# amogkam/ray_lightning_accelerators

Hardware: AMD Instinct MI355X
Metric: samples/sec (whole node) + DDP scaling eff, MNISTClassifier at 1/2/4/8 workers (higher is better)
Workload: dtype bf16; 1 GPU; model=MNISTClassifier(784-32-64-10), global_batch=32, per_gpu_batch=32, parallelism=dp1, impl=native, accelerator=ddp, launch=single, optimizer=Adam, route=single, hip_graph_steps=21, step_kernel=one-launch, step_launch=hip-graph

## Files before the change

### ray_lightning_accelerators_amd/csrc/bindings.cpp

```cpp
#include <torch/extension.h>
#include <cstdlib>
#include <map>
#include <mutex>
#include <tuple>
#include <ATen/hip/impl/HIPGuardImplMasqueradingAsCUDA.h>
#include <ATen/hip/impl/HIPStreamMasqueradingAsCUDA.h>

#include "kernels.h"
#include "comm/xgmi.h"

namespace {

using at::Tensor;
using c10::optional;

hipStream_t cur_stream(const Tensor& t) {
  return at::hip::getCurrentHIPStreamMasqueradingAsCUDA(t.get_device()).stream();
}

void check_dev(const Tensor& t, const char* name, at::ScalarType dt) {
  TORCH_CHECK(t.is_cuda(), name, " must be a GPU tensor");
  TORCH_CHECK(t.is_contiguous(), name, " must be contiguous");
  TORCH_CHECK(t.scalar_type() == dt, name, " has dtype ", t.scalar_type(), ", expected ", dt);
}
// ... 984 lines not shown
  TORCH_CHECK(conv3x3_dgrad_bn_ok(N, H, W, Cr, Co), "conv3x3_dgrad_bn_plan: unsupported shape");
  const rla::Conv3x3Geom g = conv3x3_dgrad_geom(N, H, W, Cr, Co);
  const rla::Conv3x3Instance ins = rla::conv3x3_instance(g, false);
  return {g.tm, g.wpb, g.vrows, rla::conv3x3_pieces_per_thread(g), ins.nx, ins.fixed ? 1 : 0};
}

std::vector<int64_t> conv1x1_plan(int64_t M, int64_t K, int64_t N, bool bwd) {
  TORCH_CHECK(bwd ? rla::conv1x1_bn_bwd_ok(M, (int)K, (int)N) : rla::conv1x1_stats_ok(M, (int)K, (int)N),
              "conv1x1_plan: unsupported shape");
  const rla::Conv1x1Plan p = rla::conv1x1_stats_plan(M, (int)N, bwd);
  return {p.tnw, p.gy, p.gx, p.tiles_per_blk, rla::conv1x1_variant((int)K, p)};
}

int64_t stem_grid(int64_t N, int64_t H, int64_t W) {
  const rla::StemGeom g{(int)N, (int)H, (int)W, (int)((H - 1) / 2 + 1), (int)((W - 1) / 2 + 1)};
  TORCH_CHECK(rla::stem_ok(g), "stem_grid: unsupported shape");
  return rla::stem_grid(g);
}

Tensor dp_pack_roundtrip(Tensor x, int64_t tag) {
  TORCH_CHECK(x.is_cuda() && x.scalar_type() == at::kFloat && x.is_contiguous(), "x: contiguous fp32 on the GPU");
  Tensor y = at::empty_like(x);
  TORCH_CHECK(rla::dp_pack_roundtrip(x.data_ptr<float>(), y.data_ptr<float>(), x.numel(), (int)tag, cur_stream(x)) == 0,
              "dp_pack_roundtrip: bad arguments");
  return y;
}

}

PYBIND11_MODULE(TORCH_EXTENSION_NAME, m) {
  m.doc() = "gfx950 HIP kernels of ray_lightning_accelerators_amd";
  m.def("adam_step", &adam_step, "fused Adam over a flat fp32 arena");
  m.def("sgd_step", &sgd_step, "fused SGD (momentum/nesterov/wd) over a flat fp32 arena");
  m.def("multi_copy", &multi_copy, "multi-tensor copy/scale/cast via a chunk table");
  m.def("scale_", &scale_, "in-place scale of an fp32 arena");
  m.def("sumsq", &sumsq, "sum of squares of an fp32 arena");
  m.def("mlp_train_step", &mlp_train_step, "fused MNIST-MLP forward+backward(+Adam) step",
        py::arg("x_u8"), py::arg("x_f32"), py::arg("labels"), py::arg("order"), py::arg("counters"),
        py::arg("n_batches"), py::arg("B"), py::arg("L1"), py::arg("L2"), py::arg("params"),
        py::arg("grads"), py::arg("exp_avg"), py::arg("exp_avg_sq"), py::arg("stats"),
        py::arg("accumulate_grad"), py::arg("apply_adam"), py::arg("advance_step"), py::arg("lr"),
        py::arg("beta1"), py::arg("beta2"), py::arg("eps"), py::arg("weight_decay"), py::arg("lr_t"),
        py::arg("adamw"), py::arg("stamps") = py::none());
  m.def("mlp_eval", &mlp_eval, "fused MNIST-MLP forward + NLL/accuracy");
  m.def("mlp3", &mlp3, "fused MNIST-MLP step v3 (pipelined layer 1): kind 0 step, 1 head, 2 tail-grad, "
        "3 tail-adam, 4 prime, 5 step with the in-kernel xGMI exchange, 6 one-launch step (B <= 32)");
  m.def("dp_pack_roundtrip", &dp_pack_roundtrip, "packed DP exchange wire form of fp32 pairs, encoded + decoded");
  m.def("mlp3_hand_words", [](int64_t l1, int64_t l2) { return rla::mlp3_hand_words((int)l1, (int)l2); });
  m.def("mlp3_hand_layout", []() {
    const rla::MLP3HandLayout h = rla::mlp3_hand_layout();
    py::dict d;
    d["ack"] = h.ack; d["err"] = h.err; d["sat"] = h.sat; d["nonfinite"] = h.nonfinite;
    d["last_step"] = h.last_step; d["words"] = h.words;
    return d;
  });
  m.def("mlp3_h1_copies", [](int64_t l1) { return rla::mlp3_h1_copies((int)l1); },
        "H1pre copies per ring slot of the v3 step (the layer-1 partials' atomic fan-in is split over them)");
  m.def("mlp3_dp_area_floats", []() { return rla::comm::kDpUnitAreaFloats; },
        "aux receive-area stride (floats) of the one-launch step's packed / owner protocols");
  m.def("mlp_adam", &mlp_adam, "MLP arena Adam + bf16 shadow refresh (update=False: refresh only)");
  m.def("mlp_shadow_size", [](int64_t l1, int64_t l2) { return rla::mlp_shadow_layout((int)l1, (int)l2).total; });
  m.def("mlp_supported", [](int64_t a, int64_t b) { return rla::mlp_supported((int)a, (int)b); });
  m.def("mlp_param_count", &mlp_param_count);
  m.def("bn_partial", &bn_partial, "fused BN: per-block partial sums (mode 0 fwd stats, 1 bwd dz/dz*x)",
        py::arg("x"), py::arg("y"), py::arg("dy"), py::arg("C"), py::arg("mode"), py::arg("relu"), py::arg("nbt"),
        py::arg("dy2") = py::none(), py::arg("ss") = py::none(), py::arg("dout") = py::none(),
        py::arg("pool_arg") = py::none(), py::arg("pool_geo") = std::vector<int64_t>{});
  m.def("bn_finalize", &bn_finalize, "fused BN: mean/invstd/scale/shift + running stats from partials",
        py::arg("part"), py::arg("count"), py::arg("weight"), py::arg("bias"), py::arg("running_mean"),
        py::arg("running_var"), py::arg("nbt"), py::arg("momentum"), py::arg("eps"), py::arg("nbt_pending") = false);
  m.def("bn_bwd_finalize", &bn_bwd_finalize, "fused BN backward: dgamma/dbeta + dx coefficients");
  m.def("bn_apply", &bn_apply, "fused BN apply: y = act(x*scale + shift (+res))", py::arg("x"), py::arg("scale"),
        py::arg("shift"), py::arg("res"), py::arg("relu"), py::arg("y"), py::arg("nbt_inc") = py::none());
  m.def("conv1x1_stats", &conv1x1_stats, "1x1 conv forward on MFMA + BatchNorm partial sums of its output",
        py::arg("x"), py::arg("w"), py::arg("pre_ss") = py::none(), py::arg("nbt_inc") = py::none());
  m.def("conv1x1_pre_ok", [](int64_t M, int64_t K, int64_t N) { return rla::conv1x1_pre_ok(M, (int)K, (int)N); });
  m.def("conv1x1_bn_bwd", &conv1x1_bn_bwd,
        "1x1 conv input gradient fused with the previous BatchNorm's backward partial -> (d, part)");
  m.def("conv1x1_bn_bwd_ok", [](int64_t M, int64_t K, int64_t N) { return rla::conv1x1_bn_bwd_ok(M, (int)K, (int)N); });
  m.def("conv1x1_stats_ok", [](int64_t M, int64_t K, int64_t N) { return rla::conv1x1_stats_ok(M, (int)K, (int)N); });
  m.def("maxpool_fwd", &maxpool_fwd,
        "NHWC bf16 max pool -> (y, one-byte window argmax); bn_ss: pool bf16(relu(x * scale + shift)) instead",
        py::arg("x"), py::arg("k"), py::arg("s"), py::arg("pad"), py::arg("bn_ss") = py::none(),
        py::arg("nbt_inc") = py::none());
  m.def("strided_add_", &strided_add_, "d[:, :, ::s, ::s] += g in place over NHWC bf16 rows (fp32 add)");
  m.def("gap_bwd", &gap_bwd, "global average pool backward over NHWC rows (16-byte stores)");
  m.def("maxpool_bwd", &maxpool_bwd, "NHWC bf16 max pool backward (gather through the argmax bytes)");
  m.def("bn_bwd_apply", &bn_bwd_apply, "fused BN backward apply: dx (+ dres = relu-masked dy)", py::arg("x"),
        py::arg("y"), py::arg("dy"), py::arg("coef"), py::arg("relu"), py::arg("dx"), py::arg("dres"),
        py::arg("dy2") = py::none(), py::arg("ss") = py::none(), py::arg("pool_arg") = py::none(),
        py::arg("pool_geo") = std::vector<int64_t>{});
  m.def("conv_wgrad", &conv_wgrad, "NHWC bf16 conv weight gradient on MFMA -> fp32 [Cout, KH, KW, Cin]",
        py::arg("dy"), py::arg("x"), py::arg("N"), py::arg("H"), py::arg("W"), py::arg("Cin"), py::arg("OH"),
        py::arg("OW"), py::arg("Cout"), py::arg("KH"), py::arg("KW"), py::arg("sh"), py::arg("sw"), py::arg("ph"),
        py::arg("pw"), py::arg("splits") = 0, py::arg("algo") = 0, py::arg("pre_ss") = py::none());
  m.def("conv_wgrad_plan", &conv_wgrad_plan, "the wgrad kernel's (kind, wa, wb, splits, rows_per_split)",
        py::arg("N"), py::arg("H"), py::arg("W"), py::arg("Cin"), py::arg("OH"), py::arg("OW"), py::arg("Cout"),
        py::arg("KH"), py::arg("KW"), py::arg("sh"), py::arg("sw"), py::arg("ph"), py::arg("pw"),
        py::arg("splits") = 0, py::arg("algo") = 0);
  m.def("set_plan_cus", [](int64_t n) { rla::set_plan_cus((int)std::min<int64_t>(std::max<int64_t>(n, 0), 1 << 20)); },
        "pin the CU count the persistent conv kernels' work splits are planned for (process-wide; n <= 0: the "
        "device's); the tests use it to run production per-workgroup geometry on small tensors",
        py::arg("n"));
  m.def("plan_cus", []() { return (int64_t)rla::plan_cus(); }, "the effective planning CU count");
  m.def("conv3x3_plan", &conv3x3_plan, "the 3x3 kernel's (tm, wpb, vrows, pieces_per_thread, nx, fixed)", py::arg("N"),
        py::arg("H"), py::arg("W"), py::arg("Cin"), py::arg("Cout"), py::arg("flip") = false,
// ... 38 lines not shown
```

### ray_lightning_accelerators_amd/csrc/kernels.h

```cpp
#pragma once
#include <hip/hip_runtime.h>
#include <stdint.h>

namespace rla {

struct AdamArgs {
  float* p;
  const float* g;
  float* m;
  float* v;
  uint16_t* p_bf16;
  int64_t n;
  float lr, beta1, beta2, eps, weight_decay, grad_scale;
  int adamw, maximize;
  const int64_t* step_ptr;
  int64_t host_step;
  const float* lr_ptr;
};

struct SGDArgs {
  float* p;
  const float* g;
  float* buf;
  uint16_t* p_bf16;
// ... 143 lines not shown
  int B, L1, L2;
  const float* params;
  float* logits;
  float* out;
  int partials;
};

struct MLP3Args {
  const uint8_t* x_u8;
  const int64_t* labels;
  const int64_t* order;
  int64_t order_stride;
  int64_t* counters;
  int64_t n_batches;
  int B, L1, L2;
  float* params;
  float* grads;
  float* exp_avg;
  float* exp_avg_sq;
  uint16_t* shadow;
  uint16_t* dh1t;
  uint16_t* xring;
  int* h1pre;
  uint16_t* act;
  int* yring;
  float* stats;
  int stats_ring;
  float* head_part;
  int apply_adam;
  int advance_step;
  float lr, beta1, beta2, eps, weight_decay, grad_scale;
  const float* lr_ptr;
  int adamw;
  int64_t* stamps;
  char* dp_regions[8];
  uint32_t* dp_gen;
  int* dp_err;
  int64_t dp_stride;
  int64_t dp_spin;
  int dp_rank, dp_world;
  int dp_lite;
  int dp_proto;
  int dp_loop;
  unsigned long long* hand;
  int64_t hand_spin;
};
enum MLP3Kind { kMLP3Step = 0, kMLP3Head = 1, kMLP3TailGrad = 2, kMLP3TailAdam = 3, kMLP3Prime = 4,
                kMLP3StepDP = 5, kMLP3Step1 = 6, kMLP3Step1DP = 7 };
int64_t mlp3_hand_words(int L1, int L2);
struct MLP3HandLayout {
  int ack, err, sat, nonfinite, last_step, words;
};
MLP3HandLayout mlp3_hand_layout();
int launch_mlp3(const MLP3Args& a, int kind, hipStream_t stream);

int mlp3_act_rows(int L1, int L2);
int mlp3_h1_copies(int L1);
int dp_pack_roundtrip(const float* x, float* y, int64_t n, int tag, hipStream_t stream);

int launch_mlp_train_step(const MLPStepArgs& a, hipStream_t stream);
int launch_mlp_eval(const MLPEvalArgs& a, hipStream_t stream);
bool mlp_supported(int L1, int L2);
int launch_mlp_adam(const MLPAdamArgs& a, hipStream_t stream);

}

namespace rla {
struct WgradGeom {
  int N, H, W, Cin;
  int OH, OW, Cout;
  int KH, KW, sh, sw, ph, pw;
};
struct WgradPlan {
  int kind;
  int wa, wb;
  int splits;
  int64_t rows_per_split;
};
WgradPlan wgrad_plan(const WgradGeom& g, int splits, int algo = 0);
void launch_wgrad(const uint16_t* dy, const uint16_t* x, float* out, float* part, const WgradGeom& g,
                  const WgradPlan& p, hipStream_t stream, const float* pre_ss = nullptr);

struct Conv3x3Geom {
  int N, H, W, Cin, Cout;
  int vrows;
  int tm;
  int wpb;
};
int plan_cus();
void set_plan_cus(int n);
int conv3x3_wpb(int N, int H, int W, int Cout);
int conv3x3_pick_tm(int N, int H, int W, int Cout);
int conv3x3_vrows(const Conv3x3Geom& g);
int conv3x3_pieces_per_thread(const Conv3x3Geom& g);
bool conv3x3_ok(const Conv3x3Geom& g);
struct Conv3x3Instance {
  int nx;
  bool fixed;
};
Conv3x3Instance conv3x3_instance(const Conv3x3Geom& g, bool pre);
bool conv3x3_pre_ok(const Conv3x3Geom& g);
bool conv3x3_bwd_ok(const Conv3x3Geom& g);
bool launch_conv3x3(const uint16_t* x, const uint16_t* w, uint16_t* y, const Conv3x3Geom& g, bool flip,
                    hipStream_t stream, float* part = nullptr, const float* pre_ss = nullptr,
                    int64_t* nbt_inc = nullptr, const uint16_t* bwd_x = nullptr);

// ... 26 lines not shown
```

### ray_lightning_accelerators_amd/csrc/mlp_common.h

```cpp
#pragma once
#include <math.h>

#include "common.h"

namespace rla {
namespace mlp {

constexpr int kD = 784;
constexpr int kNC = 10;
constexpr int kTiles = kD / 16;

template <int L1, int L2>
struct Off {
  static constexpr int64_t W1 = 0, B1 = (int64_t)L1 * kD, W2 = B1 + L1, B2 = W2 + (int64_t)L2 * L1,
                           W3 = B2 + L2, B3 = W3 + kNC * L2, NP = B3 + kNC;
  static constexpr int64_t W2T = (NP + 7) / 8 * 8, W3T = W2T + (int64_t)L1 * L2;
};

struct AdamScal {
  float lr, step_size, bc2_sqrt, beta1, beta2, eps, wd;
  int adamw;
};

__device__ __forceinline__ void adam_scalars(AdamScal& o, int64_t t, float lr, float b1, float b2, float eps,
                                             float wd, int adamw) {
  const double bc1 = 1.0 - pow((double)b1, (double)t);
  const double bc2 = 1.0 - pow((double)b2, (double)t);
  o.lr = lr;
  o.step_size = (float)((double)lr / bc1);
  o.bc2_sqrt = (float)sqrt(bc2);
  o.beta1 = b1; o.beta2 = b2; o.eps = eps; o.wd = wd; o.adamw = adamw;
}

__device__ __forceinline__ float adam1(float p, float g, float& m, float& v, const AdamScal& o) {
#pragma clang fp contract(off)
  if (o.wd != 0.f) {
    if (o.adamw) p = p * (1.f - o.lr * o.wd);
    else g = fmaf(o.wd, p, g);
  }
  m = fmaf(1.f - o.beta1, g - m, m);
  v = fmaf(1.f - o.beta2, g * g, v * o.beta2);
  const float denom = sqrtf(v) / o.bc2_sqrt + o.eps;
  return fmaf(-o.step_size, m / denom, p);
}

typedef __attribute__((address_space(3))) bf16x4 lds_bf16x4;
__device__ __forceinline__ bf16x4 tr_read(const __bf16* p) {
  return __builtin_amdgcn_ds_read_tr16_b64_v4bf16((lds_bf16x4*)(p));
}
__device__ __forceinline__ bf16x8 ld8(const __bf16* p) { return *reinterpret_cast<const bf16x8*>(p); }
__device__ __forceinline__ float4 ld4(const float* p) { return *reinterpret_cast<const float4*>(p); }

__device__ __forceinline__ void u8x16_to_bf16(const uint4 v, bf16x8& lo, bf16x8& hi) {
  const uint32_t wd[4] = {v.x, v.y, v.z, v.w};
  constexpr float inv255 = 1.0f / 255.0f;
#pragma unroll
  for (int j = 0; j < 4; ++j) {
    lo[j] = (__bf16)((float)((wd[0] >> (8 * j)) & 0xffu) * inv255);
    lo[4 + j] = (__bf16)((float)((wd[1] >> (8 * j)) & 0xffu) * inv255);
    hi[j] = (__bf16)((float)((wd[2] >> (8 * j)) & 0xffu) * inv255);
    hi[4 + j] = (__bf16)((float)((wd[3] >> (8 * j)) & 0xffu) * inv255);
  }
}

}
}
```

### ray_lightning_accelerators_amd/csrc/mlp_step3.hip

```cpp
#include <cfloat>

#include "common.h"
#include "kernels.h"
#include "mlp_common.h"
#include "comm/xgmi.h"

namespace rla {
namespace {

using namespace mlp;
using comm::kDpMaxBlocks;
using comm::kXgmiFlagBytes;
using comm::kXgmiMaxRanks;

constexpr int kThreads = 512;
constexpr int kWaves = 8;
constexpr int kDZS = 40;
constexpr int kXSS = 24;
constexpr int kBMax = 256;
constexpr int kCnt = 5;
constexpr int kHeadRows = 32;

enum TailMode { kFused = 0, kGrad = 1, kAdam = 2, kPrime = 3, kFusedDP = 4 };

// ... 24 lines not shown
};

template <int BC, int L1, int L2>
constexpr bool fits3() {
  return Cfg3<BC, L1, L2>::total + 256 <= 160 * 1024;
}

__device__ __forceinline__ __bf16 relu_bf(float x) { return (__bf16)fmaxf(x, 0.f); }

constexpr float kFix = 1048576.0f;
constexpr float kFixSat = 33554432.0f;
__device__ __forceinline__ unsigned f32_to_fixed(float x) {
  return (unsigned)__float2int_rn(fminf(fmaxf(x * kFix, -kFixSat), kFixSat));
}
__device__ __forceinline__ float fixed_to_f32(int q) { return (float)q * (1.0f / 1048576.0f); }

template <int L1>
struct H1Copies {
  static constexpr int G = L1 <= 64 ? 2 : 1;
};

__device__ __forceinline__ void gather_tile(const MLP3Args& a, int kt, int64_t ob, int64_t cursor,
                                            int64_t dst_slot, int nthreads) {
  const int tid = threadIdx.x;
  const int B = a.B, Bp = (B + 31) / 32 * 32;
  const int64_t* idx = a.order + ob * a.order_stride + cursor * B;
  __bf16* dst = reinterpret_cast<__bf16*>(a.xring) + (dst_slot * kTiles + kt) * (int64_t)Bp * 16;
  for (int b = tid; b < Bp; b += nthreads) {
    bf16x8 lo = zero8(), hi = zero8();
    if (b < B) u8x16_to_bf16(*reinterpret_cast<const uint4*>(a.x_u8 + idx[b] * kD + kt * 16), lo, hi);
    *reinterpret_cast<bf16x8*>(dst + b * 16) = lo;
    *reinterpret_cast<bf16x8*>(dst + b * 16 + 8) = hi;
  }
  if (kt == 0)
    for (int b = tid; b < Bp; b += nthreads) a.yring[dst_slot * Bp + b] = b < B ? (int)a.labels[idx[b]] : -1;
}

__device__ __forceinline__ int64_t ld_state(const int64_t* p, int i) {
  return ((const __attribute__((address_space(4))) int64_t*)(p))[i];
}

__device__ __forceinline__ void stamp_max(const MLP3Args& a, int k) {
  if (a.stamps && threadIdx.x == 0)
    atomicMax(reinterpret_cast<unsigned long long*>(a.stamps + k),
              (unsigned long long)__builtin_amdgcn_s_memrealtime());
}

constexpr int kSeq = 10;
constexpr int kHandAck = 0, kHandErr = 16, kHandWords = 32;

constexpr int kHandSat = 17, kHandNonFinite = 18, kHandLastStep = 19;
static_assert(kHandLastStep < kHandWords, "health words inside the hand buffer");
constexpr float kH1Sat = 32.0f;

struct H1Health {
  unsigned sat = 0u, bad = 0u;
};

__device__ __forceinline__ void h1_check(H1Health& h, const f32x4& d, int row0, int B) {
  const bool trouble = !(fabsf(d[0]) <= kH1Sat) | !(fabsf(d[1]) <= kH1Sat) | !(fabsf(d[2]) <= kH1Sat) |
                       !(fabsf(d[3]) <= kH1Sat);
  if (__builtin_amdgcn_ballot_w64(trouble) == 0ull) return;
#pragma unroll
  for (int i = 0; i < 4; ++i) {
    const float m = fabsf(d[i]);
    const bool real = row0 + i < B, finite = m <= FLT_MAX;
    h.bad += (unsigned)__builtin_popcountll(__builtin_amdgcn_ballot_w64(real && !finite));
    h.sat += (unsigned)__builtin_popcountll(__builtin_amdgcn_ballot_w64(real && finite && m > kH1Sat));
  }
}

__device__ __forceinline__ void h1_report(const MLP3Args& a, const H1Health& h, int64_t step) {
  if ((h.sat | h.bad) == 0u || !a.hand) return;
  if ((threadIdx.x & 63) == 0) {
    if (h.sat)
      __hip_atomic_fetch_add(a.hand + kHandSat, (unsigned long long)h.sat, __ATOMIC_RELAXED, __HIP_MEMORY_SCOPE_AGENT);
    if (h.bad)
      __hip_atomic_fetch_add(a.hand + kHandNonFinite, (unsigned long long)h.bad, __ATOMIC_RELAXED,
                             __HIP_MEMORY_SCOPE_AGENT);
    __hip_atomic_fetch_max(a.hand + kHandLastStep, (unsigned long long)step, __ATOMIC_RELAXED,
                           __HIP_MEMORY_SCOPE_AGENT);
  }
}

struct RepPre {
  bool active;
  int64_t si;
  int kt;
  uint4 xn;
  int64_t yn;
  uint32_t raw;
};

struct NoHook {
  __device__ void operator()() const {}
};

__device__ __forceinline__ void dma_lds16(const void* gsrc, uint32_t lds) {
  uint32_t keep;
  asm volatile("s_mov_b32 %0, m0\n\ts_mov_b32 m0, %2\n\ts_nop 0\n\tglobal_load_lds_dwordx4 %1, off\n\ts_mov_b32 m0, %0"
               : "=&s"(keep)
               : "v"(gsrc), "s"(lds)
               : "memory");
}
__device__ __forceinline__ void dma_lds4(const void* gsrc, uint32_t lds) {
  uint32_t keep;
// ... 558 lines not shown
      row = REP ? L->dh2t + (e - L1) * L->ts : ACT + (int64_t)(A::DH2T + e - L1) * Bp;
      r.gi[0] = O::B2 + (e - L1);
    } else {
      row = REP ? L->dzt + (e - L1 - L2) * L->ts : ACT + (int64_t)(A::DZT + e - L1 - L2) * Bp;
      r.gi[0] = O::B3 + (e - L1 - L2);
    }
    if (setup) {
      r.kind = 2;
      r.valid[0] = true;
      if (prefetch_adam) { r.pv[0] = a.params[r.gi[0]]; r.mv[0] = a.exp_avg[r.gi[0]]; r.vv[0] = a.exp_avg_sq[r.gi[0]]; }
    }
    if (!compute) return;
    float s8[8] = {0.f, 0.f, 0.f, 0.f, 0.f, 0.f, 0.f, 0.f};

    for (int b0 = 0; b0 < Bp; b0 += 32) {
      bf16x8 v[4];
#pragma unroll
      for (int q = 0; q < 4; ++q) v[q] = ld8(row + b0 + 8 * q);
#pragma unroll
      for (int q = 0; q < 4; ++q)
#pragma unroll
        for (int j = 0; j < 8; ++j) s8[j] += (float)v[q][j];
    }
    r.v[0] = ((s8[0] + s8[1]) + (s8[2] + s8[3])) + ((s8[4] + s8[5]) + (s8[6] + s8[7]));
  }
}

template <int L1, int L2>
__device__ __forceinline__ void small_finalize(const MLP3Args& a, bool adam, const SmallRes& r, const AdamScal& o) {
  using O = Off<L1, L2>;
  if (r.kind < 0) return;
  __bf16* SHW = reinterpret_cast<__bf16*>(a.shadow);
  bf16x4 sh4;
#pragma unroll
  for (int i = 0; i < 4; ++i) {
    sh4[i] = (__bf16)0.f;
    if (!r.valid[i]) continue;
    if (adam) {
      float m_ = r.mv[i], v_ = r.vv[i];
      const float p_ = adam1(r.pv[i], r.v[i], m_, v_, o);
      a.params[r.gi[i]] = p_;
      a.exp_avg[r.gi[i]] = m_;
      a.exp_avg_sq[r.gi[i]] = v_;
      SHW[r.gi[i]] = (__bf16)p_;
      sh4[i] = (__bf16)p_;
    } else {
      a.grads[r.gi[i]] = r.v[i];
    }
  }
  if (adam && r.kind == 0) *reinterpret_cast<bf16x4*>(SHW + O::W2T + (int64_t)r.colv * L2 + r.rowv) = sh4;
  if (adam && r.kind == 1) *reinterpret_cast<bf16x4*>(SHW + O::W3T + (int64_t)r.colv * 16 + r.rowv) = sh4;
}

template <int L1, int L2>
__device__ __forceinline__ void small_store(const MLP3Args& a, const SmallRes& r, bool store_mv) {
  using O = Off<L1, L2>;
  if (r.kind < 0) return;
  __bf16* SHW = reinterpret_cast<__bf16*>(a.shadow);
  bf16x4 sh4;
#pragma unroll
  for (int i = 0; i < 4; ++i) {
    sh4[i] = (__bf16)0.f;
    if (!r.valid[i]) continue;
    a.params[r.gi[i]] = r.v[i];
    if (store_mv) {
      a.exp_avg[r.gi[i]] = r.mv[i];
      a.exp_avg_sq[r.gi[i]] = r.vv[i];
    }
    SHW[r.gi[i]] = (__bf16)r.v[i];
    sh4[i] = (__bf16)r.v[i];
  }
  if (r.kind == 0) *reinterpret_cast<bf16x4*>(SHW + O::W2T + (int64_t)r.colv * L2 + r.rowv) = sh4;
  if (r.kind == 1) *reinterpret_cast<bf16x4*>(SHW + O::W3T + (int64_t)r.colv * 16 + r.rowv) = sh4;
}

__device__ __forceinline__ uint32_t* dp_flag(char* region, int slot, int blk, int src) {
  return reinterpret_cast<uint32_t*>(region) + ((size_t)slot * kDpMaxBlocks + blk) * kXgmiMaxRanks + src;
}
__device__ __forceinline__ float* dp_data(char* region, int slot, int src, int64_t stride) {
  return reinterpret_cast<float*>(region + kXgmiFlagBytes) + ((int64_t)slot * kXgmiMaxRanks + src) * stride;
}

__device__ __forceinline__ int dp_begin(const MLP3Args& a, uint32_t* sh_gen) {
  if (threadIdx.x == 0) *sh_gen = a.dp_gen[blockIdx.x] + 1u;
  __syncthreads();
  return (int)(*sh_gen & 1u);
}

__device__ __forceinline__ void dp_signal_and_wait(const MLP3Args& a, uint32_t gen, int slot, int* sh_fail) {
  if (a.dp_lite) {
    const int tid = threadIdx.x, blk = blockIdx.x;
    asm volatile("s_waitcnt vmcnt(0)" ::: "memory");
    __syncthreads();
    if (tid < 64) {
      if (tid == 0) *sh_fail = 0;
      __builtin_amdgcn_fence(__ATOMIC_RELEASE, "");
      asm volatile("s_waitcnt vmcnt(0)" ::: "memory");
      if (tid < a.dp_world)
        __hip_atomic_store(dp_flag(a.dp_regions[tid], slot, blk, a.dp_rank), gen, __ATOMIC_RELAXED,
                           __HIP_MEMORY_SCOPE_SYSTEM);
      if (tid < a.dp_world) {
        uint32_t* f = dp_flag(a.dp_regions[a.dp_rank], slot, blk, tid);
        int64_t spins = 0;
        while (__hip_atomic_load(f, __ATOMIC_RELAXED, __HIP_MEMORY_SCOPE_SYSTEM) != gen) {
          if (++spins > a.dp_spin) {
            *sh_fail = 1;
// ... 542 lines not shown
  static constexpr int NSMALL = (NTASK + kWaves - 1) / kWaves;
  static constexpr size_t oImg = C::total;
  static constexpr size_t oTile = oImg + (size_t)(2 * L2 + L1) * C::TS * 2;
  static constexpr size_t oRaw = oTile + (size_t)(2 * 32 + L1) * kXSS * 2 + 64;
  static constexpr size_t lds = oRaw + kPreRawBytes;
};
static_assert(One<128, 256>::lds <= 160 * 1024, "one-launch LDS budget");

__device__ __forceinline__ void one_wait_acks(const MLP3Args& a, int64_t seq, int* sh_fail) {
  if (threadIdx.x == 0) {
    const long long target = (long long)(seq + 1) * (long long)gridDim.x;
    const long long* ack = reinterpret_cast<const long long*>(a.hand + kHandAck);
    int64_t n = 0;
    *sh_fail = 0;
    while (__hip_atomic_load(ack, __ATOMIC_RELAXED, __HIP_MEMORY_SCOPE_AGENT) < target) {
      if (++n > a.hand_spin) {
        *sh_fail = 1;
        __hip_atomic_store(a.hand + kHandErr, 1ull, __ATOMIC_RELAXED, __HIP_MEMORY_SCOPE_AGENT);
        if (a.dp_err) __hip_atomic_store(a.dp_err, 2, __ATOMIC_RELAXED, __HIP_MEMORY_SCOPE_SYSTEM);
        break;
      }
      __builtin_amdgcn_s_sleep(2);
    }
  }
  asm volatile("" ::: "memory");
  __syncthreads();
}

template <int L1, int L2, int DPP, int NW = 8>
__global__ __launch_bounds__(kThreads) void mlp3_one_kernel(MLP3Args a) {
  constexpr bool DP = DPP >= 0;
  using C = typename One<L1, L2>::C;
  using S = SmallTasks<L1, L2>;
  constexpr int TN1 = L1 / 16, Bp = 32;
  __shared__ __attribute__((aligned(16))) char smem[One<L1, L2>::lds];
  __shared__ int sh_fail;
  __bf16* sH2T = (__bf16*)(smem + One<L1, L2>::oImg);
  __bf16* sDH2T = sH2T + L2 * C::TS;
  __bf16* sDH1T = sDH2T + L2 * C::TS;
  __bf16* sX = (__bf16*)(smem + One<L1, L2>::oTile);
  __bf16* sXn = sX + Bp * kXSS;
  __bf16* sW = sXn + Bp * kXSS;
  AdamScal* sh_o = reinterpret_cast<AdamScal*>(sW + L1 * kXSS);
  const int tid = threadIdx.x, lane = tid & 63, w = tid >> 6, r16 = lane & 15, g = lane >> 4;
  const int blk = blockIdx.x;
  const bool tile = blk >= 1 && blk <= kTiles, small = blk > kTiles;
  const int kt = blk - 1;
  if (a.stamps && blk == 1 && tid == 0) a.stamps[8] = __builtin_amdgcn_s_memrealtime();
  stamp_max(a, 13);

  const int64_t c0 = ld_state(a.counters, 0), cursor = ld_state(a.counters, 1);
  const int64_t slot = ld_state(a.counters, 3), ob = ld_state(a.counters, 4);
  const int64_t seq = ld_state(a.counters, kSeq);
  const uint32_t dgen = DP ? dp_gen_now(a) : 0u;
  const int B = a.B;

  const int m = w * 16 + r16, pix = kt * 16 + 4 * g;
  const bool mw = tile && w < TN1;
  const int64_t gidx = mw ? (int64_t)m * kD + pix : 0;
  F4 p4, m4, v4;
  SmallRes r;
  r.kind = -1;
  const int task = (blk - 1 - kTiles) * kWaves + w;
  if (small) small_compute<L1, L2, true>(a, true, task, r);
  const float lr_now = a.lr_ptr ? ((const __attribute__((address_space(4))) float*)(a.lr_ptr))[0] : a.lr;
  __bf16* XR = reinterpret_cast<__bf16*>(a.xring);
  constexpr int64_t tile_elems = (int64_t)Bp * 16;
  const int xb = lane & 31;
  bf16x8 xc0, xc1;
  RepPre pre;
  pre.active = tile && w == PreWave<L1>::wave;
  pre.raw = (uint32_t)(uintptr_t)(const __attribute__((address_space(3))) void*)(smem + One<L1, L2>::oRaw);
  pre.kt = tile ? kt : 0;
  pre.xn = make_uint4(0u, 0u, 0u, 0u);
  pre.yn = -1;
  int64_t nc = cursor + 1, nob = ob;
  if (nc >= a.n_batches) { nc = 0; nob ^= 1; }
  const int kt_c = tile ? kt : 0;
  auto hook = [&]() {
    pre.si = a.order[nob * a.order_stride + nc * B + (xb < B ? xb : 0)];
    const __bf16* cur = XR + (slot * kTiles + kt_c) * tile_elems + xb * 16;
    xc0 = ld8(cur);
    xc1 = ld8(cur + 8);
    p4 = *reinterpret_cast<const F4*>(a.params + gidx);
    m4 = *reinterpret_cast<const F4*>(a.exp_avg + gidx);
    v4 = *reinterpret_cast<const F4*>(a.exp_avg_sq + gidx);
  };
  if (tid == 0 && blk > 0)
    adam_scalars(*sh_o, a.advance_step ? c0 + 1 : c0, lr_now, a.beta1, a.beta2, a.eps, a.weight_decay, a.adamw);

  head_body<32, L1, L2, false, true>(a, smem, &pre, hook);

  if (a.stamps && blk == 1 && tid == 0) a.stamps[9] = __builtin_amdgcn_s_memrealtime();
  stamp_max(a, 12);

  if (tile) {
    if (w == 0 && lane < 32) {
      *reinterpret_cast<bf16x8*>(sX + xb * kXSS) = xc0;
      *reinterpret_cast<bf16x8*>(sX + xb * kXSS + 8) = xc1;
    }
    __syncthreads();
    if (a.stamps && blk == 1 && tid == 0) a.stamps[7] = __builtin_amdgcn_s_memrealtime();
    bf16x4 w4;
    f32x4 acc = {0.f, 0.f, 0.f, 0.f};
    if (mw) {
      const int q = r16 >> 2, pp = r16 & 3;
      const bf16x4 lo = tr_read(sX + (8 * g + q) * kXSS + 4 * pp);
      const bf16x4 hi = tr_read(sX + (8 * g + 4 + q) * kXSS + 4 * pp);
      const bf16x8 afrag = __builtin_shufflevector(lo, hi, 0, 1, 2, 3, 4, 5, 6, 7);
      acc = mfma16(afrag, ld8(sDH1T + m * C::TS + 8 * g), acc);
    }
    bool adam_done = false, store_mv = true;
    if constexpr (DP) {
      const uint32_t gen = dgen;
      const int dslot = (int)(gen & 1u);
      int fail = 0;
      if (mw) {
        if constexpr (DPP == 0) {
#pragma unroll
          for (int i = 0; i < 4; ++i) dp_push_gran(a, dslot, gidx + i, acc[i], gen);
#pragma unroll
          for (int i = 0; i < 4; ++i) acc[i] = dp_sum_gran(a, dslot, gidx + i, gen, &fail) * a.grad_scale;
        } else {
          float v[4] = {acc[0], acc[1], acc[2], acc[3]};
          const int unit = blk * kWaves + w;
          if constexpr (DPP == 1) {
            dp_packed_exchange<NW>(a, unit, gen, v, a.grad_scale, &fail);
          } else {
            const AdamScal o = *sh_o;
            store_mv = dp_owner_step<NW>(a, unit, dp_task_owner(a, kt), gen, v, a.grad_scale, &fail,
                                     [&](float (&x)[4]) {
#pragma unroll
                                       for (int i = 0; i < 4; ++i) x[i] = adam1(p4.v[i], x[i], m4.v[i], v4.v[i], o);
                                     });
            store_mv = store_mv || a.dp_loop;
            adam_done = true;
#pragma unroll
            for (int i = 0; i < 4; ++i) p4.v[i] = v[i];
          }
#pragma unroll
          for (int i = 0; i < 4; ++i) acc[i] = v[i];
        }
      }
// ... 39 lines not shown
    if (mw) {
      constexpr int G = H1Copies<L1>::G;
      unsigned* h1 = reinterpret_cast<unsigned*>(a.h1pre + ((slot ^ 1) * G + kt % G) * (int64_t)Bp * L1);
      const bf16x8 bfrag = (g < 2) ? ld8(sW + (w * 16 + r16) * kXSS + 8 * g) : zero8();
      H1Health health;
#pragma unroll
      for (int mt = 0; mt < Bp / 16; ++mt) {
        const bf16x8 afrag = (g < 2) ? ld8(sXn + (mt * 16 + r16) * kXSS + 8 * g) : zero8();
        const f32x4 d = mfma16(afrag, bfrag, f32x4{0.f, 0.f, 0.f, 0.f});
        unsigned* dst = h1 + (int64_t)((mt * TN1 + w) * 4) * 64 + lane;
#pragma unroll
        for (int i = 0; i < 4; ++i) atomicAdd(dst + i * 64, f32_to_fixed(d[i]));
        h1_check(health, d, mt * 16 + 4 * g, B);
      }
      h1_report(a, health, c0 + 1);
    }
    if (a.stamps && blk == 1 && tid == 0) a.stamps[10] = __builtin_amdgcn_s_memrealtime();
    stamp_max(a, 5);
  } else if (small) {
    const RepLds L{(const __bf16*)(smem + C::oH1T), sH2T, sDH2T, (const __bf16*)(smem + C::odZT), sDH1T, C::TS};
    small_compute<L1, L2, true>(a, true, task, r, &L);
    bool adam_done = false, store_mv = true;
    if constexpr (DP) {
      const uint32_t gen = dgen;
      const int dslot = (int)(gen & 1u);
      int fail = 0;
      if constexpr (DPP == 0) {
#pragma unroll
        for (int i = 0; i < 4; ++i)
          if (r.valid[i]) dp_push_gran(a, dslot, r.gi[i], r.v[i], gen);
#pragma unroll
        for (int i = 0; i < 4; ++i)
          if (r.valid[i]) r.v[i] = dp_sum_gran(a, dslot, r.gi[i], gen, &fail) * a.grad_scale;
      } else if (task < S::NTASK) {
        float v[4] = {r.v[0], r.v[1], r.v[2], r.v[3]};
        const int unit = blk * kWaves + w;
        if constexpr (DPP == 1) {
          dp_packed_exchange<NW>(a, unit, gen, v, a.grad_scale, &fail);
        } else {
          const AdamScal o = *sh_o;
          store_mv = dp_owner_step<NW>(a, unit, dp_task_owner(a, kTiles + task), gen, v, a.grad_scale, &fail,
                                   [&](float (&x)[4]) {
#pragma unroll
                                     for (int i = 0; i < 4; ++i) x[i] = adam1(r.pv[i], x[i], r.mv[i], r.vv[i], o);
                                   });
          store_mv = store_mv || a.dp_loop;
          adam_done = true;
        }
#pragma unroll
        for (int i = 0; i < 4; ++i) r.v[i] = v[i];
      }
      dp_end_nosync(a, gen, fail);
    }
    one_wait_acks(a, seq, &sh_fail);
    if (adam_done) small_store<L1, L2>(a, r, store_mv);
    else small_finalize<L1, L2>(a, true, r, *sh_o);
    stamp_max(a, 6);
  } else {
    HeadStats hs{0.f, 0.f, 0.f};
    if (w == 0) hs = head_stats((const float*)(smem + C::oZ));
    one_wait_acks(a, seq, &sh_fail);
    uint4* z = reinterpret_cast<uint4*>(a.h1pre + slot * H1Copies<L1>::G * (int64_t)Bp * L1);
    for (int i = tid; i < H1Copies<L1>::G * Bp * L1 / 4; i += kThreads) z[i] = make_uint4(0u, 0u, 0u, 0u);
    if (tid == 0) {
      const int64_t t = c0 + 1;
      int64_t nc = cursor + 1, nob = ob;
      if (nc >= a.n_batches) { nc = 0; nob ^= 1; }
      const int64_t st[kCnt] = {a.advance_step ? t : t - 1, nc, cursor, slot ^ 1, nob};
      for (int k = 0; k < kCnt; ++k) a.counters[k] = a.counters[kCnt + k] = st[k];
      a.counters[kSeq] = seq + 1;
      if (a.stats) {
        float* sr = a.stats + (int)((t - 1) % (a.stats_ring > 0 ? a.stats_ring : 1)) * 4;
        sr[0] = hs.loss * (1.f / (float)B);
        sr[1] = hs.correct;
        sr[2] = hs.cnt;
        sr[3] = (float)t;
      }
      if (a.stamps) a.stamps[4] = __builtin_amdgcn_s_memrealtime();
    }
  }
  stamp_max(a, 11);
}

template <int L1, int L2>
int dispatch3(const MLP3Args& a, int kind, hipStream_t stream) {
  constexpr int kOneGrid = 1 + kTiles + One<L1, L2>::NSMALL;
  if (kind == kMLP3Step1) {
    if (a.B > 32 || !a.hand || kOneGrid > 256) return -5;
    hipLaunchKernelGGL((mlp3_one_kernel<L1, L2, -1>), dim3(kOneGrid), dim3(kThreads), 0, stream, a);
    return 0;
  }
  if (kind == kMLP3Step1DP) {
    if (a.B > 32 || !a.hand || kOneGrid > kDpMaxBlocks || a.dp_world < 1 || a.dp_world > kXgmiMaxRanks ||
        !a.dp_gen || !a.dp_err || a.dp_proto < 0 || a.dp_proto > 2)
      return -6;
    if (a.dp_proto == 0 ? (a.dp_lite != 2 || a.dp_stride < 2 * Off<L1, L2>::NP) : a.dp_stride < comm::kDpUnitAreaFloats)
      return -7;
    const dim3 g(kOneGrid), b(kThreads);
    const int nw = a.dp_world <= 2 ? 2 : (a.dp_world <= 4 ? 4 : 8);
    if (a.dp_proto == 0) hipLaunchKernelGGL((mlp3_one_kernel<L1, L2, 0>), g, b, 0, stream, a);
    else if (a.dp_proto == 1 && nw == 2) hipLaunchKernelGGL((mlp3_one_kernel<L1, L2, 1, 2>), g, b, 0, stream, a);
    else if (a.dp_proto == 1 && nw == 4) hipLaunchKernelGGL((mlp3_one_kernel<L1, L2, 1, 4>), g, b, 0, stream, a);
    else if (a.dp_proto == 1) hipLaunchKernelGGL((mlp3_one_kernel<L1, L2, 1, 8>), g, b, 0, stream, a);
    else if (nw == 2) hipLaunchKernelGGL((mlp3_one_kernel<L1, L2, 2, 2>), g, b, 0, stream, a);
    else if (nw == 4) hipLaunchKernelGGL((mlp3_one_kernel<L1, L2, 2, 4>), g, b, 0, stream, a);
    else hipLaunchKernelGGL((mlp3_one_kernel<L1, L2, 2, 8>), g, b, 0, stream, a);
    return 0;
  }
  constexpr int NT = 64 * (L1 / 16);
  if (kind == kMLP3StepDP && (a.dp_world < 1 || a.dp_world > kXgmiMaxRanks || !a.dp_gen || !a.dp_err ||
                              a.dp_stride < Off<L1, L2>::NP || kTiles + SmallTasks<L1, L2>::NBLK > kDpMaxBlocks))
    return -3;
  if (kind == kMLP3Step || kind == kMLP3Head || kind == kMLP3StepDP) {
    const int nchunks = (a.B + kHeadRows - 1) / kHeadRows;
    if (nchunks > 1 && !a.head_part) return -4;
    if (nchunks > 1)
      hipLaunchKernelGGL((mlp3_head_kernel<kHeadRows, L1, L2, true>), dim3(nchunks + kTiles), dim3(kThreads), 0, stream, a);
    else
      hipLaunchKernelGGL((mlp3_head_kernel<kHeadRows, L1, L2, false>), dim3(1 + kTiles), dim3(kThreads), 0, stream, a);
  }
  int mode = -1, grid = kTiles;
  if (kind == kMLP3Step) { mode = kFused; grid += SmallTasks<L1, L2>::NBLK; }
  else if (kind == kMLP3StepDP) { mode = kFusedDP; grid += SmallTasks<L1, L2>::NBLK; }
  else if (kind == kMLP3TailGrad) { mode = kGrad; grid += SmallTasks<L1, L2>::NBLK; }
  else if (kind == kMLP3Prime) mode = kPrime;
  else if (kind == kMLP3TailAdam) {
    mode = kAdam;
    const int64_t nsmall = Off<L1, L2>::NP - Off<L1, L2>::B1;
    int extra = (int)((nsmall + NT - 1) / NT);
    grid += extra < 64 ? extra : 64;
  }
  if (mode >= 0) hipLaunchKernelGGL((mlp3_tail_kernel<L1, L2>), dim3(grid), dim3(NT), 0, stream, a, mode);
  return 0;
}

static_assert(fits3<kHeadRows, 128, 256>(), "v3 head LDS budget");

__global__ void dp_pack_roundtrip_kernel(const float* x, float* y, int64_t n, uint32_t tag) {
  const int64_t i = (int64_t)blockIdx.x * blockDim.x + threadIdx.x;
  if (2 * i + 1 < n + 1) {
    const float v0 = x[2 * i], v1 = 2 * i + 1 < n ? x[2 * i + 1] : 0.f;
    const u64 w = pk2(v0, v1, tag);
    y[2 * i] = ((uint32_t)w & 3u) == tag ? pk_lo(w) : __builtin_nanf("");
    if (2 * i + 1 < n) y[2 * i + 1] = pk_hi(w);
  }
}

}

int dp_pack_roundtrip(const float* x, float* y, int64_t n, int tag, hipStream_t stream) {
  if (n <= 0 || tag < 0 || tag > 3) return -1;
  const int64_t pairs = (n + 1) / 2;
  hipLaunchKernelGGL(dp_pack_roundtrip_kernel, dim3((unsigned)((pairs + 255) / 256)), dim3(256), 0, stream, x, y, n,
                     (uint32_t)tag);
  return 0;
}

int mlp3_act_rows(int L1, int L2) { return L1 + 2 * L2 + 16; }
int mlp3_h1_copies(int L1) { return L1 <= 64 ? H1Copies<64>::G : H1Copies<128>::G; }
int64_t mlp3_hand_words(int, int) { return kHandWords; }
MLP3HandLayout mlp3_hand_layout() {
  return {kHandAck, kHandErr, kHandSat, kHandNonFinite, kHandLastStep, kHandWords};
}

int launch_mlp3(const MLP3Args& a, int kind, hipStream_t stream) {
  if (a.B > kBMax || a.B < 1) return -2;
#define RLA_CASE(a1, a2) if (a.L1 == a1 && a.L2 == a2) return dispatch3<a1, a2>(a, kind, stream);
  RLA_CASE(32, 32) RLA_CASE(32, 64) RLA_CASE(32, 128) RLA_CASE(32, 256)
  RLA_CASE(64, 64) RLA_CASE(64, 128) RLA_CASE(64, 256)
  RLA_CASE(128, 64) RLA_CASE(128, 128) RLA_CASE(128, 256)
#undef RLA_CASE
  return -1;
}

}
```

### ray_lightning_accelerators_amd/ops/fused_mlp.py

```python
from __future__ import annotations

import math
from typing import Dict, Optional, Sequence, Tuple

import torch
import torch.nn.functional as F

from . import require, use_native

IN_FEATURES = 784
NUM_CLASSES = 10
SUPPORTED = {(32, 32), (32, 64), (32, 128), (32, 256), (64, 64), (64, 128), (64, 256),
             (128, 64), (128, 128), (128, 256)}


def mlp_param_count(L1: int, L2: int) -> int:
    return L1 * IN_FEATURES + L1 + L2 * L1 + L2 + NUM_CLASSES * L2 + NUM_CLASSES


def mlp_supported(L1: int, L2: int) -> bool:
    return (int(L1), int(L2)) in SUPPORTED


def mlp_unpack(flat: torch.Tensor, L1: int, L2: int) -> Dict[str, torch.Tensor]:
# ... 101 lines not shown
def mlp_shadow_layout(L1: int, L2: int) -> Dict[str, int]:
    np_ = mlp_param_count(L1, L2)
    w2t = (np_ + 7) // 8 * 8
    w3t = w2t + L1 * L2
    return {"np": np_, "w2t": w2t, "w3t": w3t, "total": w3t + 16 * L2}


def mlp_refresh_shadow(params: torch.Tensor, shadow: torch.Tensor, L1: int, L2: int) -> None:
    if use_native(params):
        require().mlp_adam(params, params, params, params, shadow, int(L1), int(L2), 0.0, 0.9, 0.999, 1e-8, 0.0,
                           1.0, False, False, None, None)
        return
    lay = mlp_shadow_layout(L1, L2)
    v = mlp_unpack(params, L1, L2)
    with torch.no_grad():
        shadow[: lay["np"]].copy_(params)
        shadow[lay["w2t"]: lay["w3t"]].copy_(v["layer_2.weight"].t().reshape(-1))
        w3t = torch.zeros(L2, 16, dtype=params.dtype, device=params.device)
        w3t[:, :NUM_CLASSES] = v["layer_3.weight"].t()
        shadow[lay["w3t"]: lay["total"]].copy_(w3t.reshape(-1))


MLP3_STEP, MLP3_HEAD, MLP3_TAIL_GRAD, MLP3_TAIL_ADAM, MLP3_PRIME, MLP3_STEP_DP, MLP3_STEP1, MLP3_STEP1_DP = range(8)
ONE_LAUNCH_MAX_B = 32
DP_GRANULE, DP_PACKED, DP_OWNER = 0, 1, 2
DP_PROTOS = {"granule": DP_GRANULE, "packed": DP_PACKED, "owner": DP_OWNER}
DP_AREA_FLOATS = 327680


def mlp3_dp_capacity(L1: int, L2: int) -> int:
    return max(2 * mlp_param_count(L1, L2), DP_AREA_FLOATS)


def mlp3_hand_words(L1: int, L2: int) -> int:
    return 32


HAND_LAYOUT = {"ack": 0, "err": 16, "sat": 17, "nonfinite": 18, "last_step": 19, "words": 32}
_hand_layout: Optional[Dict[str, int]] = None


def mlp3_hand_layout(native: bool = True) -> Dict[str, int]:
    global _hand_layout
    if not native:
        return dict(HAND_LAYOUT)
    if _hand_layout is None:
        lay = {k: int(v) for k, v in require().mlp3_hand_layout().items()}
        if lay != HAND_LAYOUT:
            raise RuntimeError(f"hand layout of the extension {lay} differs from ops.fused_mlp.HAND_LAYOUT")
        _hand_layout = lay
    return dict(_hand_layout)


W1_TILES = IN_FEATURES // 16
H1_SAT = 32.0


def mlp3_h1_health(x_rows: torch.Tensor, w1_bf16: torch.Tensor) -> Tuple[int, int]:
    xt = x_rows.detach().cpu().to(torch.bfloat16).double().view(x_rows.size(0), W1_TILES, 16)
    wt = w1_bf16.detach().cpu().to(torch.bfloat16).double().view(w1_bf16.size(0), W1_TILES, 16)
    part = torch.einsum("bti,mti->tbm", xt, wt).float()
    mag = part.abs()
    bad = ~(mag <= torch.finfo(torch.float32).max)
    sat = (mag > H1_SAT) & ~bad
    return int(sat.sum()), int(bad.sum())


def mlp3_h1_copies(L1: int) -> int:
    return 2 if int(L1) <= 64 else 1


def mlp3_buffers(L1: int, L2: int, B: int, device) -> Dict[str, torch.Tensor]:
    bp = (B + 31) // 32 * 32
    return {
        "dh1t": torch.zeros(L1 * bp, dtype=torch.bfloat16, device=device),
        "xring": torch.zeros(2 * W1_TILES * bp * 16, dtype=torch.bfloat16, device=device),
        "h1pre": torch.zeros(2 * mlp3_h1_copies(L1) * bp * L1, dtype=torch.int32, device=device),
        "act": torch.zeros((L1 + 2 * L2 + 16) * bp, dtype=torch.bfloat16, device=device),
        "yring": torch.full((2 * bp,), -1, dtype=torch.int32, device=device),
        "counters": torch.zeros(16, dtype=torch.int64, device=device),
        "hand": torch.zeros(mlp3_hand_words(L1, L2), dtype=torch.int64, device=device),
        "head_part": torch.zeros(bp // 32 * 4, device=device),
    }


def mlp3_launch(
    kind: int,
    *,
    x_u8: torch.Tensor,
    labels: torch.Tensor,
    order: torch.Tensor,
    counters: torch.Tensor,
    n_batches: int,
    B: int,
    L1: int,
    L2: int,
    params: torch.Tensor,
    grads: torch.Tensor,
    exp_avg: torch.Tensor,
    exp_avg_sq: torch.Tensor,
    shadow: torch.Tensor,
    dh1t: torch.Tensor,
    xring: torch.Tensor,
    h1pre: torch.Tensor,
    act: torch.Tensor,
    yring: torch.Tensor,
# ... 81 lines not shown
```

Measured before the change: 4.477 million samples/s.

## Precompute Adam bias corrections for the next step and cache them in the hand buffer

The one-launch step used to compute the Adam bias-correction terms (two double-precision pow calls) serially on thread 0 of each block. The tail block now computes the next step's bc1 and sqrt(bc2) during the ack wait and stores them, keyed by step and betas, in spare words of the hand buffer. The next launch reads them back and falls back to a two-lane parallel pow (bc1 and bc2 on separate lanes) when the key misses. The small-tensor Adam update is also split so its arithmetic runs before the ack wait and only the store runs after it. This adds cross-launch state that must stay in sync when the step counter or betas change.

```diff
diff --git a/ray_lightning_accelerators_amd/csrc/bindings.cpp b/ray_lightning_accelerators_amd/csrc/bindings.cpp
--- a/ray_lightning_accelerators_amd/csrc/bindings.cpp
+++ b/ray_lightning_accelerators_amd/csrc/bindings.cpp
@@ -1060,6 +1060,12 @@
     py::dict d;
     d["ack"] = h.ack; d["err"] = h.err; d["sat"] = h.sat; d["nonfinite"] = h.nonfinite;
     d["last_step"] = h.last_step; d["words"] = h.words;
+    return d;
+  });
+  m.def("mlp3_adam_cache_layout", []() {
+    const rla::MLP3AdamCacheLayout c = rla::mlp3_adam_cache_layout();
+    py::dict d;
+    d["step"] = c.step; d["betas"] = c.betas; d["bc1"] = c.bc1; d["bc2_sqrt"] = c.bc2_sqrt;
     return d;
   });
   m.def("mlp3_h1_copies", [](int64_t l1) { return rla::mlp3_h1_copies((int)l1); },
diff --git a/ray_lightning_accelerators_amd/csrc/kernels.h b/ray_lightning_accelerators_amd/csrc/kernels.h
--- a/ray_lightning_accelerators_amd/csrc/kernels.h
+++ b/ray_lightning_accelerators_amd/csrc/kernels.h
@@ -219,6 +219,10 @@
   int ack, err, sat, nonfinite, last_step, words;
 };
 MLP3HandLayout mlp3_hand_layout();
+struct MLP3AdamCacheLayout {
+  int step, betas, bc1, bc2_sqrt;
+};
+MLP3AdamCacheLayout mlp3_adam_cache_layout();
 int launch_mlp3(const MLP3Args& a, int kind, hipStream_t stream);
 
 int mlp3_act_rows(int L1, int L2);
diff --git a/ray_lightning_accelerators_amd/csrc/mlp_common.h b/ray_lightning_accelerators_amd/csrc/mlp_common.h
--- a/ray_lightning_accelerators_amd/csrc/mlp_common.h
+++ b/ray_lightning_accelerators_amd/csrc/mlp_common.h
@@ -29,6 +29,27 @@
   o.lr = lr;
   o.step_size = (float)((double)lr / bc1);
   o.bc2_sqrt = (float)sqrt(bc2);
+  o.beta1 = b1; o.beta2 = b2; o.eps = eps; o.wd = wd; o.adamw = adamw;
+}
+
+struct AdamBias {
+  double bc1, bc2_sqrt;
+};
+
+__device__ __forceinline__ AdamBias adam_bias2(int64_t t, float b1, float b2) {
+  const bool first = (threadIdx.x & 63) == 0;
+  const double p = pow((double)(first ? b1 : b2), (double)t);
+  const int lo = __double2loint(p), hi = __double2hiint(p);
+  const double p1 = __hiloint2double(__builtin_amdgcn_readlane(hi, 0), __builtin_amdgcn_readlane(lo, 0));
+  const double p2 = __hiloint2double(__builtin_amdgcn_readlane(hi, 1), __builtin_amdgcn_readlane(lo, 1));
+  return AdamBias{1.0 - p1, sqrt(1.0 - p2)};
+}
+
+__device__ __forceinline__ void adam_scalars_bias(AdamScal& o, const AdamBias& c, float lr, float b1, float b2,
+                                                  float eps, float wd, int adamw) {
+  o.lr = lr;
+  o.step_size = (float)((double)lr / c.bc1);
+  o.bc2_sqrt = (float)c.bc2_sqrt;
   o.beta1 = b1; o.beta2 = b2; o.eps = eps; o.wd = wd; o.adamw = adamw;
 }
 
diff --git a/ray_lightning_accelerators_amd/csrc/mlp_step3.hip b/ray_lightning_accelerators_amd/csrc/mlp_step3.hip
--- a/ray_lightning_accelerators_amd/csrc/mlp_step3.hip
+++ b/ray_lightning_accelerators_amd/csrc/mlp_step3.hip
@@ -100,6 +100,12 @@
 constexpr int kHandSat = 17, kHandNonFinite = 18, kHandLastStep = 19;
 static_assert(kHandLastStep < kHandWords, "health words inside the hand buffer");
 constexpr float kH1Sat = 32.0f;
+
+constexpr int kHandAdamStep = 20, kHandAdamBetas = 21, kHandAdamBc1 = 22, kHandAdamBc2 = 23;
+static_assert(kHandAdamStep > kHandLastStep && kHandAdamBc2 < kHandWords, "cache words are spare words of hand");
+__device__ __forceinline__ unsigned long long adam_betas_key(float b1, float b2) {
+  return (unsigned long long)__float_as_uint(b1) | ((unsigned long long)__float_as_uint(b2) << 32);
+}
 
 struct H1Health {
   unsigned sat = 0u, bad = 0u;
@@ -764,6 +770,13 @@
   if (adam && r.kind == 1) *reinterpret_cast<bf16x4*>(SHW + O::W3T + (int64_t)r.colv * 16 + r.rowv) = sh4;
 }
 
+__device__ __forceinline__ void small_adam(SmallRes& r, const AdamScal& o) {
+  if (r.kind < 0) return;
+#pragma unroll
+  for (int i = 0; i < 4; ++i)
+    if (r.valid[i]) r.v[i] = adam1(r.pv[i], r.v[i], r.mv[i], r.vv[i], o);
+}
+
 template <int L1, int L2>
 __device__ __forceinline__ void small_store(const MLP3Args& a, const SmallRes& r, bool store_mv) {
   using O = Off<L1, L2>;
@@ -1412,6 +1425,10 @@
   const int64_t c0 = ld_state(a.counters, 0), cursor = ld_state(a.counters, 1);
   const int64_t slot = ld_state(a.counters, 3), ob = ld_state(a.counters, 4);
   const int64_t seq = ld_state(a.counters, kSeq);
+  const int64_t* hand_s = reinterpret_cast<const int64_t*>(a.hand);
+  const int64_t ck_step = ld_state(hand_s, kHandAdamStep), ck_betas = ld_state(hand_s, kHandAdamBetas);
+  const int64_t ck_bc1 = ld_state(hand_s, kHandAdamBc1), ck_bc2 = ld_state(hand_s, kHandAdamBc2);
+  const int64_t t_adam = a.advance_step ? c0 + 1 : c0;
   const uint32_t dgen = DP ? dp_gen_now(a) : 0u;
   const int B = a.B;
 
@@ -1445,10 +1462,17 @@
     p4 = *reinterpret_cast<const F4*>(a.params + gidx);
     m4 = *reinterpret_cast<const F4*>(a.exp_avg + gidx);
     v4 = *reinterpret_cast<const F4*>(a.exp_avg_sq + gidx);
+    if (w == 0 && blk > 0) {
+      if (t_adam > 0 && ck_step == t_adam && ck_betas == (int64_t)adam_betas_key(a.beta1, a.beta2)) {
+        if (lane == 0)
+          adam_scalars_bias(*sh_o, AdamBias{__longlong_as_double(ck_bc1), __longlong_as_double(ck_bc2)}, lr_now,
+                            a.beta1, a.beta2, a.eps, a.weight_decay, a.adamw);
+      } else if (lane < 2) {
+        const AdamBias bc = adam_bias2(t_adam, a.beta1, a.beta2);
+        if (lane == 0) adam_scalars_bias(*sh_o, bc, lr_now, a.beta1, a.beta2, a.eps, a.weight_decay, a.adamw);
+      }
+    }
   };
-  if (tid == 0 && blk > 0)
-    adam_scalars(*sh_o, a.advance_step ? c0 + 1 : c0, lr_now, a.beta1, a.beta2, a.eps, a.weight_decay, a.adamw);
-
   head_body<32, L1, L2, false, true>(a, smem, &pre, hook);
 
   if (a.stamps && blk == 1 && tid == 0) a.stamps[9] = __builtin_amdgcn_s_memrealtime();
@@ -1594,14 +1618,23 @@
       }
       dp_end_nosync(a, gen, fail);
     }
+    if (!adam_done) small_adam(r, *sh_o);
     one_wait_acks(a, seq, &sh_fail);
-    if (adam_done) small_store<L1, L2>(a, r, store_mv);
-    else small_finalize<L1, L2>(a, true, r, *sh_o);
+    small_store<L1, L2>(a, r, store_mv);
     stamp_max(a, 6);
   } else {
     HeadStats hs{0.f, 0.f, 0.f};
     if (w == 0) hs = head_stats((const float*)(smem + C::oZ));
+    const int64_t t_next = a.advance_step ? t_adam + 1 : t_adam;
+    AdamBias nbc{0.0, 0.0};
+    if (w == 1 && lane < 2) nbc = adam_bias2(t_next, a.beta1, a.beta2);
     one_wait_acks(a, seq, &sh_fail);
+    if (tid == 64) {
+      a.hand[kHandAdamStep] = (unsigned long long)t_next;
+      a.hand[kHandAdamBetas] = adam_betas_key(a.beta1, a.beta2);
+      a.hand[kHandAdamBc1] = (unsigned long long)__double_as_longlong(nbc.bc1);
+      a.hand[kHandAdamBc2] = (unsigned long long)__double_as_longlong(nbc.bc2_sqrt);
+    }
     uint4* z = reinterpret_cast<uint4*>(a.h1pre + slot * H1Copies<L1>::G * (int64_t)Bp * L1);
     for (int i = tid; i < H1Copies<L1>::G * Bp * L1 / 4; i += kThreads) z[i] = make_uint4(0u, 0u, 0u, 0u);
     if (tid == 0) {
@@ -1704,6 +1737,7 @@
 MLP3HandLayout mlp3_hand_layout() {
   return {kHandAck, kHandErr, kHandSat, kHandNonFinite, kHandLastStep, kHandWords};
 }
+MLP3AdamCacheLayout mlp3_adam_cache_layout() { return {kHandAdamStep, kHandAdamBetas, kHandAdamBc1, kHandAdamBc2}; }
 
 int launch_mlp3(const MLP3Args& a, int kind, hipStream_t stream) {
   if (a.B > kBMax || a.B < 1) return -2;
diff --git a/ray_lightning_accelerators_amd/ops/fused_mlp.py b/ray_lightning_accelerators_amd/ops/fused_mlp.py
--- a/ray_lightning_accelerators_amd/ops/fused_mlp.py
+++ b/ray_lightning_accelerators_amd/ops/fused_mlp.py
@@ -177,6 +177,17 @@
     return dict(_hand_layout)
 
 
+ADAM_CACHE_LAYOUT = {"step": 20, "betas": 21, "bc1": 22, "bc2_sqrt": 23}
+
+
+def mlp3_adam_cache_layout(native: bool = True) -> Dict[str, int]:
+    if native:
+        lay = {k: int(v) for k, v in require().mlp3_adam_cache_layout().items()}
+        if lay != ADAM_CACHE_LAYOUT:
+            raise RuntimeError(f"Adam cache layout of the extension {lay} differs from ops.fused_mlp.ADAM_CACHE_LAYOUT")
+    return dict(ADAM_CACHE_LAYOUT)
+
+
 W1_TILES = IN_FEATURES // 16
 H1_SAT = 32.0
 
```

After: 4.715 million samples/s, median of 6. +5.3%, better.
